# virajmehta/vae-training

Hardware: AMD Instinct MI355X
Metric: ELBO train-step samples/sec (higher is better)
Workload: dtype f32; 1 GPU; M: linear-padding dd3 pad9 (D=12) L=20 linear enc/dec -tdv eps=-1 lr=1e-3 (seed_linpadding_expts.sh:1); batch_per_gpu=65536, global_batch=65536, data_dim=12, latent_dim=20, params=533, parallelism=dp1, grad_exchange=none, launch=direct library call x2395 steps (arguments marshalled once), input_batches=48

## Files before the change

### vae_training_amd/csrc/linear_moments.hip

```cpp
#include <stdlib.h>

#include <type_traits>

#include "comm_dev.h"
#include "rng_dev.h"
#include "vaek_internal.h"

namespace vaek {

using f32x4 = __attribute__((ext_vector_type(4))) float;
using d2 = __attribute__((ext_vector_type(2))) double;
typedef __attribute__((address_space(3))) void lds_void_t;
typedef const __attribute__((address_space(1))) void glb_void_t;

constexpr int LNT = 512, LNW = LNT / 64;
constexpr int kLinMaxPersist = 64;
constexpr int kLinCarry = 2, kLinSlots = kLinMaxPersist + kLinCarry;
struct LinWindow { int first, count; };
struct LinWindows { LinWindow stream, reduce, update; };
constexpr LinWindows lin_windows(int K, int j) {
    const int s0 = kLinMaxPersist * j, s1 = s0 + kLinMaxPersist < K ? s0 + kLinMaxPersist : K;
    const bool last = s1 == K;
    const int r0 = s0 >= 1 ? s0 - 1 : 0, u0 = s0 >= 2 ? s0 - 2 : 0;
    return LinWindows{{s0, s1 - s0}, {r0, (last ? K : s1 - 1) - r0}, {u0, (last ? K : s1 - 2) - u0}};
}
constexpr int lin_launches(int K) { return (K + kLinMaxPersist - 1) / kLinMaxPersist; }
constexpr bool lin_windows_ok(int K) {
    int s = 0, r = 0, u = 0;
    for (int j = 0; j < lin_launches(K); ++j) {
        const LinWindows w = lin_windows(K, j);
        if (w.stream.first != s || w.reduce.first != r || w.update.first != u) return false;
        if (w.stream.count < 1 || w.stream.count > kLinMaxPersist || w.reduce.count < 1 || w.update.count < 1) return false;
        s += w.stream.count; r += w.reduce.count; u += w.update.count;
        if (r > s || u > r || s - w.update.first > kLinSlots) return false;
    }
    return s == K && r == K && u == K;
}
static_assert(lin_windows_ok(1) && lin_windows_ok(2) && lin_windows_ok(64) && lin_windows_ok(65) && lin_windows_ok(66) && lin_windows_ok(128) &&
              lin_windows_ok(129) && lin_windows_ok(130) && lin_windows_ok(960), "launch windows of a vaek_train_steps call");
static_assert(lin_windows(64, 0).update.count == 64 && lin_windows(130, 1).update.first == 62 && lin_windows(130, 1).reduce.first == 63 &&
              lin_windows(130, 2).update.count == 4, "launch windows of a vaek_train_steps call");
constexpr int kLinReduceSets = 1;
constexpr int kLinReduceWgs = 24;

constexpr int kLinCommBanks = 4;
struct LinComm { unsigned long long* peer[kMaxWorld]; int world, rank, ng2; };

constexpr int kLinShards = 8, kLinShardStride = 32;
struct LinPtrs { const float* x[64]; const float* z1[64]; const float* z2[64]; };
struct LinArgs {
    int has_update, n_reduce, n_stream;
    int B, D, L, ntiles, T;
    const float* x; const float* z1; const float* z2; float* partial_out;
    const float* partial_in; double* M_out;
    const double* M_in;
    int persistent, n_steps, sets;
    int n_red, n_str, slot_upd, slot_red, slot_str;
    int d_red, d_str;
    float* partial_base; double* M_base;
    unsigned* cnt_stream; unsigned* cnt_reduce; unsigned* status;
    float* params; float* grads; float* m; float* v; int32_t* step_dev; float lr;
    float inv_bt, eps_cli, rows, rows_over_bt; int off_eps, P;
    float* loss_hist; long long loss_hist_cap;
    int stagger;
    LinComm comm;
};

#ifndef VAEK_LIN_ABL
#define VAEK_LIN_ABL 0
#endif
#ifdef VAEK_LIN_STAMPS
#ifdef VAEK_LIN_FOUR_BLOCK_TU
static __device__ unsigned long long* g_lin_stamp_buf = nullptr;
#else
__device__ unsigned long long* g_lin_stamp_buf = nullptr;
#endif
int lin_stamps_four(unsigned long long* buf);
#define LIN_STAMP(i)                                                                                         \
    do {                                                                                                     \
        if (VAEK_LIN_STAMPS == 2) break;          \
        __builtin_amdgcn_sched_barrier(0);                                                                   \
        unsigned long long _t;                                                                               \
        unsigned long long _r;                                                                               \
        asm volatile("s_waitcnt vmcnt(0) lgkmcnt(0)\n\ts_memtime %0\n\ts_memrealtime %1\n\ts_waitcnt lgkmcnt(0)" : "=s"(_t), "=s"(_r)::"memory"); \
        if (g_lin_stamp_buf && threadIdx.x == 0) { g_lin_stamp_buf[i] = _t; g_lin_stamp_buf[16 + (i)] = _r; } \
        __builtin_amdgcn_sched_barrier(0);                                                                   \
    } while (0)
#define LIN_NOW(v)                                                                                           \
    do {                                                                                                     \
        __builtin_amdgcn_sched_barrier(0);                                                                   \
        if (VAEK_LIN_STAMPS == 2) asm volatile("s_memrealtime %0\n\ts_waitcnt lgkmcnt(0)" : "=s"(v)::"memory");             \
        else asm volatile("s_waitcnt vmcnt(0) lgkmcnt(0)\n\ts_memrealtime %0\n\ts_waitcnt lgkmcnt(0)" : "=s"(v)::"memory"); \
        __builtin_amdgcn_sched_barrier(0);                                                                   \
    } while (0)
#define LIN_NOWQ(v)                                     \
    do {                                                                                                     \
        __builtin_amdgcn_sched_barrier(0);                                                                   \
        asm volatile("s_memrealtime %0\n\ts_waitcnt lgkmcnt(0)" : "=s"(v)::"memory");                        \
        __builtin_amdgcn_sched_barrier(0);                                                                   \
    } while (0)
#define LIN_PUT(i, v) do { if (g_lin_stamp_buf && threadIdx.x == 0) g_lin_stamp_buf[i] = (v); } while (0)
#define LIN_PUTMAX(i, v) do { if (g_lin_stamp_buf && threadIdx.x == 0) atomicMax(&g_lin_stamp_buf[i], (v)); } while (0)
#else
#define LIN_STAMP(i) do {} while (0)
#define LIN_NOW(v) do {} while (0)
#define LIN_NOWQ(v) do {} while (0)
#define LIN_PUT(i, v) do {} while (0)
#define LIN_PUTMAX(i, v) do {} while (0)
#endif

__device__ __forceinline__ void lin_glds16(const void* gsrc, void* lds_wave_base) {
    __builtin_amdgcn_global_load_lds((glb_void_t*)gsrc, (lds_void_t*)lds_wave_base, 16, 0, 0);
}
template <int N> __device__ __forceinline__ void lin_wait_vmcnt() { asm volatile("s_waitcnt vmcnt(%0)" ::"n"(N) : "memory"); }
__device__ __forceinline__ void lin_barrier() { asm volatile("s_waitcnt lgkmcnt(0)\n\ts_barrier" ::: "memory"); }
__device__ __forceinline__ void lin_wait_vmcnt_upto(int n) {
    switch (n) {
        case 1: lin_wait_vmcnt<1>(); break;   case 2: lin_wait_vmcnt<2>(); break;   case 3: lin_wait_vmcnt<3>(); break;
        case 4: lin_wait_vmcnt<4>(); break;   case 5: lin_wait_vmcnt<5>(); break;   case 6: lin_wait_vmcnt<6>(); break;
        case 7: lin_wait_vmcnt<7>(); break;   case 8: lin_wait_vmcnt<8>(); break;   case 9: lin_wait_vmcnt<9>(); break;
        case 10: lin_wait_vmcnt<10>(); break; case 11: lin_wait_vmcnt<11>(); break; case 12: lin_wait_vmcnt<12>(); break;
        case 13: lin_wait_vmcnt<13>(); break; case 14: lin_wait_vmcnt<14>(); break; case 15: lin_wait_vmcnt<15>(); break;
        case 16: lin_wait_vmcnt<16>(); break; case 17: lin_wait_vmcnt<17>(); break; case 18: lin_wait_vmcnt<18>(); break;
        case 19: lin_wait_vmcnt<19>(); break; case 20: lin_wait_vmcnt<20>(); break;
        default: lin_wait_vmcnt<0>(); break;
    }
}

__device__ __host__ constexpr int lin_blk(int NB, int b1, int b2) { return b1 * NB - b1 * (b1 - 1) / 2 + (b2 - b1); }

__device__ __forceinline__ void st_sc1(float* p, float v) { __hip_atomic_store(p, v, __ATOMIC_RELAXED, __HIP_MEMORY_SCOPE_AGENT); }
__device__ __forceinline__ void st_sc1(double* p, double v) { __hip_atomic_store(p, v, __ATOMIC_RELAXED, __HIP_MEMORY_SCOPE_AGENT); }
__device__ __forceinline__ float ld_sc1(const float* p) { return __hip_atomic_load(p, __ATOMIC_RELAXED, __HIP_MEMORY_SCOPE_AGENT); }
__device__ __forceinline__ double ld_sc1(const double* p) { return __hip_atomic_load(p, __ATOMIC_RELAXED, __HIP_MEMORY_SCOPE_AGENT); }

__device__ __forceinline__ void lin_wait_count(const unsigned* cnt, unsigned target, unsigned* status, unsigned tag) {
    if (threadIdx.x == 0) {
        unsigned spins = 0, seen;
        while ((seen = __hip_atomic_load(cnt, __ATOMIC_RELAXED, __HIP_MEMORY_SCOPE_AGENT)) < target) {
            __builtin_amdgcn_s_sleep(16);
            if ((++spins & 1023u) == 0) {
                if (__hip_atomic_load(status, __ATOMIC_RELAXED, __HIP_MEMORY_SCOPE_AGENT)) break;
                if (spins > (1u << 21)) {
                    unsigned expect = 0;
                    __hip_atomic_compare_exchange_strong(status, &expect, 0x80000000u | tag | (seen & 0xffffu), __ATOMIC_RELAXED,
                                                         __ATOMIC_RELAXED, __HIP_MEMORY_SCOPE_AGENT);
                    break;
                }
            }
        }
    }
    __syncthreads();
}

__device__ __forceinline__ void lin_wait_shards(const unsigned* cnt, unsigned target, unsigned* status, unsigned tag) {
    if (threadIdx.x == 0) {
        unsigned spins = 0, seen;
        for (;;) {
            unsigned v[kLinShards];
#pragma unroll
            for (int k = 0; k < kLinShards; ++k) v[k] = __hip_atomic_load(cnt + k * kLinShardStride, __ATOMIC_RELAXED, __HIP_MEMORY_SCOPE_AGENT);
            seen = 0;
#pragma unroll
            for (int k = 0; k < kLinShards; ++k) seen += v[k];
            if (seen >= target) break;
            __builtin_amdgcn_s_sleep(4);
            if ((++spins & 1023u) == 0) {
                if (__hip_atomic_load(status, __ATOMIC_RELAXED, __HIP_MEMORY_SCOPE_AGENT)) break;
                if (spins > (1u << 21)) {
                    unsigned expect = 0;
                    __hip_atomic_compare_exchange_strong(status, &expect, 0x80000000u | tag | (seen & 0xffffu), __ATOMIC_RELAXED,
                                                         __ATOMIC_RELAXED, __HIP_MEMORY_SCOPE_AGENT);
                    break;
                }
            }
        }
    }
    __syncthreads();
}

__device__ __forceinline__ double lin_sum_over_ranks(const LinComm& c, unsigned epoch, int o, double v, unsigned* status) {
    const unsigned long long bits = (unsigned long long)__double_as_longlong(v), tag = (unsigned long long)epoch << 32;
    const long long bank = (long long)(epoch & (kLinCommBanks - 1)) * c.world * c.ng2;
    for (int p = 0; p < c.world; ++p) {
        unsigned long long* q = c.peer[p] + bank + (long long)c.rank * c.ng2 + 2 * o;
        __hip_atomic_store(q, tag | (bits & 0xffffffffull), __ATOMIC_RELAXED, __HIP_MEMORY_SCOPE_SYSTEM);
        __hip_atomic_store(q + 1, tag | (bits >> 32), __ATOMIC_RELAXED, __HIP_MEMORY_SCOPE_SYSTEM);
    }
    const unsigned long long* own = c.peer[c.rank] + bank + 2 * o;
    double sum = 0.0;
    unsigned spins = 0;
    bool dead = false;
    for (int r = 0; r < c.world; ++r) {
        unsigned long long lo = 0, hi = 0;
        for (;;) {
            lo = __hip_atomic_load(own + (long long)r * c.ng2, __ATOMIC_RELAXED, __HIP_MEMORY_SCOPE_SYSTEM);
            hi = __hip_atomic_load(own + (long long)r * c.ng2 + 1, __ATOMIC_RELAXED, __HIP_MEMORY_SCOPE_SYSTEM);
            if (((unsigned)(lo >> 32) == epoch && (unsigned)(hi >> 32) == epoch) || dead) break;
            __builtin_amdgcn_s_sleep(8);
            if ((++spins & 1023u) == 0) {
                if (__hip_atomic_load(status, __ATOMIC_RELAXED, __HIP_MEMORY_SCOPE_AGENT)) dead = true;
                else if (spins > (1u << 21)) {
                    unsigned expect = 0;
                    __hip_atomic_compare_exchange_strong(status, &expect, 0x80000000u | (3u << 28) | ((unsigned)r << 16) | (epoch & 0xffffu),
                                                         __ATOMIC_RELAXED, __ATOMIC_RELAXED, __HIP_MEMORY_SCOPE_AGENT);
                    dead = true;
                }
            }
        }
        sum += __longlong_as_double((long long)((hi << 32) | (lo & 0xffffffffull)));
    }
    return sum;
}

struct LinTile {
    int nz1, nx, np, oX, oZ2, bytes;
    __device__ __host__ LinTile(int D, int L, int T) {
        nz1 = (L * 4 * T + 1023) >> 10; nx = (D * 4 * T + 1023) >> 10; np = nz1 + 2 * nx;
        oX = (nz1 << 10) + 80;
        oZ2 = oX + (nx << 10); bytes = (oZ2 + (nx << 10) + 255) & ~255;
    }
};

__device__ __forceinline__ void lin_issue_piece(const LinArgs& a, const LinTile& tl, const float* x, const float* z1, const float* z2,
                                                int tile, int p, char* slot, int lane) {
    const float* src; int cols, idx, lds_off;
    if (p < tl.nz1) { src = z1; cols = a.L; idx = p; lds_off = 0; }
    else if (p < tl.nz1 + tl.nx) { src = x; cols = a.D; idx = p - tl.nz1; lds_off = tl.oX; }
    else { src = z2; cols = a.D; idx = p - tl.nz1 - tl.nx; lds_off = tl.oZ2; }
    const long long tot = (long long)a.B * cols * 4, base = (long long)tile * a.T * cols * 4;
    const long long last = min(tot & ~15ll, base + (long long)a.T * cols * 4) - 16;
    long long off = base + idx * 1024 + lane * 16;
    off = off <= last ? off : last;
    lin_glds16(reinterpret_cast<const char*>(src) + off, slot + lds_off + idx * 1024);
}

struct LinTileSrc {
    const char *z1, *x, *z2; long long baseL, lastL, baseD, lastD; char* slot; bool on;
    __device__ __forceinline__ void prepare(const LinArgs& a, const float* px, const float* pz1, const float* pz2, int tile, char* slot_) {
        auto uni = [](const float* q) {
            const unsigned long long u = (unsigned long long)q;
            return reinterpret_cast<const char*>((unsigned long long)(unsigned)__builtin_amdgcn_readfirstlane((unsigned)u) |
                                                 ((unsigned long long)(unsigned)__builtin_amdgcn_readfirstlane((unsigned)(u >> 32)) << 32));
        };
        z1 = uni(pz1); x = uni(px); z2 = uni(pz2); slot = slot_; on = true;
        const long long rows = (long long)tile * a.T;
        const long long totL = (long long)a.B * a.L * 4, totD = (long long)a.B * a.D * 4;
        baseL = rows * a.L * 4; baseD = rows * a.D * 4;
        lastL = min(totL & ~15ll, baseL + (long long)a.T * a.L * 4) - 16;
        lastD = min(totD & ~15ll, baseD + (long long)a.T * a.D * 4) - 16;
    }
    __device__ __forceinline__ void issue(const LinTile& tl, int p, int lane) const {
        const char* src; long long base, last; int idx, lds_off;
        if (p < tl.nz1) { src = z1; base = baseL; last = lastL; idx = p; lds_off = 0; }
        else if (p < tl.nz1 + tl.nx) { src = x; base = baseD; last = lastD; idx = p - tl.nz1; lds_off = tl.oX; }
        else { src = z2; base = baseD; last = lastD; idx = p - tl.nz1 - tl.nx; lds_off = tl.oZ2; }
        long long off = base + idx * 1024 + lane * 16;
        off = off <= last ? off : last;
        lin_glds16(src + off, slot + lds_off + idx * 1024);
    }
#pragma clang diagnostic push
#pragma clang diagnostic ignored "-Winline-asm"
    __device__ __forceinline__ void issue_tile(const LinTile& tl, int lw, int NLW, int lane) const {
        auto region = [&](const char* src, long long base, long long last, int n, int lds_off) __attribute__((always_inline)) {
            const long long b2 = base <= last ? base : last;
            const char* sbase = src + b2;
            const unsigned lastrel = (unsigned)(last - b2), degenerate = base <= last ? 0xffffffffu : 0u;
            const unsigned m0_0 = (unsigned)(size_t)(lds_void_t*)(slot + lds_off);
            for (int idx = lw; idx < n; idx += NLW) {
                unsigned off = ((unsigned)idx * 1024u + (unsigned)lane * 16u) & degenerate;
                off = off <= lastrel ? off : lastrel;
                asm volatile("s_mov_b32 m0, %2\n\ts_nop 0\n\tglobal_load_lds_dwordx4 %0, %1" ::"v"(off), "s"(sbase), "s"(m0_0 + (unsigned)idx * 1024u) : "memory", "m0");
            }
        };
        region(z1, baseL, lastL, tl.nz1, 0);
        region(x, baseD, lastD, tl.nx, tl.oX);
        region(z2, baseD, lastD, tl.np - tl.nz1 - tl.nx, tl.oZ2);
    }
#pragma clang diagnostic pop
};

__device__ __forceinline__ void lin_fix_ragged(const LinArgs& a, const LinTile& tl, const float* x, const float* z1, const float* z2,
                                               int tile, char* slot, int t) {
    const int T = a.T;
    const long long row0 = (long long)tile * T;
    const int valid = (int)min((long long)T, (long long)a.B - row0), D = a.D, L = a.L;
    if (valid < T) {
        auto patch_tail = [&](const float* src, int cols, int lds_off) {
            const long long tot = (long long)a.B * cols * 4, full = tot & ~15ll, base = row0 * cols * 4;
            if (t < (int)((tot - full) / 4) && full >= base) reinterpret_cast<float*>(slot + lds_off)[(full - base) / 4 + t] = src[full / 4 + t];
        };
        patch_tail(z1, L, 0); patch_tail(x, D, tl.oX); patch_tail(z2, D, tl.oZ2);
        for (int e = valid * L + t; e < T * L; e += LNT) reinterpret_cast<float*>(slot)[e] = 0.f;
        for (int e = valid * D + t; e < T * D; e += LNT) { reinterpret_cast<float*>(slot + tl.oX)[e] = 0.f; reinterpret_cast<float*>(slot + tl.oZ2)[e] = 0.f; }
    }
    lin_barrier();
}
__device__ __forceinline__ void lin_write_vcol(float* v, int T, int valid, int t) {
    for (int r = t; r < T; r += LNT) v[r] = r < valid ? 1.f : 0.f;
}

__device__ __forceinline__ void st_sc1_x4(float* p, f32x4 v) {
    asm volatile("global_store_dwordx4 %0, %1, off sc1\n\ts_nop 1" ::"v"(p), "v"(v) : "memory");
}

constexpr int lin_scratch_bytes(int NB) { return LNW * (NB * (NB + 1) / 2) * 1024; }
constexpr int lin_ring_scratch_bytes(int NB) { return NB == 3 ? lin_scratch_bytes(NB) : lin_scratch_bytes(NB) / 2; }
constexpr int kLinCW = 4;
template <int NB, int JT, int CW, typename Hook>
__device__ __forceinline__ void lin_tile_products(const LinArgs& a, const LinTile& tl, const char* smem, int slot_off, int v_off, int c_off,
                                                  f32x4 (&acc)[NB * (NB + 1) / 2], int lane, int wave, Hook&& hook) {
    constexpr int NBLK = NB * (NB + 1) / 2;
    const int g = lane >> 4, D = a.D, L = a.L;
    int fb[NB], fs[NB];
#pragma unroll
    for (int u = 0; u < NB; ++u) {
        const int f = 16 * u + (lane & 15);
        if (f < L) { fb[u] = slot_off + f * 4; fs[u] = L * 4; }
        else if (f < L + D) { fb[u] = slot_off + tl.oX + (f - L) * 4; fs[u] = D * 4; }
        else if (f < L + 2 * D) { fb[u] = slot_off + tl.oZ2 + (f - L - D) * 4; fs[u] = D * 4; }
        else if (f == L + 2 * D) { fb[u] = v_off; fs[u] = 4; }
        else { fb[u] = c_off; fs[u] = 0; }
    }
#pragma unroll
    for (int k = 0; k < NBLK; ++k) acc[k] = f32x4{0.f, 0.f, 0.f, 0.f};
    const int J = JT ? JT : a.T / (4 * CW), wbase = (a.T / CW) * wave, jfull = J & ~3;
    auto products = [&](const float (&op)[NB]) __attribute__((always_inline)) {
        int k = 0;
#pragma unroll
        for (int b1 = 0; b1 < NB; ++b1)
#pragma unroll
            for (int b2 = b1; b2 < NB; ++b2, ++k) {
                if (VAEK_LIN_ABL & 2) acc[k][0] += op[b1] * op[b2];
                else acc[k] = __builtin_amdgcn_mfma_f32_16x16x4f32(op[b1], op[b2], acc[k], 0, 0, 0);
            }
    };
    if constexpr (JT > 0) {
        constexpr int JF = JT & ~3;
        int cur[NB], fs13[NB], tail[NB];
#pragma unroll
        for (int u = 0; u < NB; ++u) {
            cur[u] = fb[u] + (wbase + 4 * g) * fs[u]; fs13[u] = 13 * fs[u];
            tail[u] = fb[u] + (wbase + 4 * JF + (JT - JF) * g) * fs[u];
        }
        float op[JT][NB];
        auto fetch = [&](int j) __attribute__((always_inline)) {
#pragma unroll
            for (int u = 0; u < NB; ++u) {
                if (j == JF) cur[u] = tail[u];
                op[j][u] = *reinterpret_cast<const float*>(smem + cur[u]);
                cur[u] += (j < JF && (j & 3) == 3) ? fs13[u] : fs[u];
            }
        };
        fetch(0);
        if (JT > 1) fetch(1);
#pragma unroll
        for (int j = 0; j < JT; ++j) {
            if (j + 2 < JT) fetch(j + 2);
            hook(j);
            __builtin_amdgcn_sched_barrier(0);
            products(op[j]);
            __builtin_amdgcn_sched_barrier(0);
        }
    } else {
        float op[2][NB];
        auto fetch = [&](int set, int j) __attribute__((always_inline)) {
            const int sample = wbase + (j < jfull ? 16 * (j >> 2) + (j & 3) + 4 * g : 4 * jfull + (j - jfull) + (J - jfull) * g);
#pragma unroll
            for (int u = 0; u < NB; ++u) op[set][u] = *reinterpret_cast<const float*>(smem + fb[u] + sample * fs[u]);
        };
        fetch(0, 0);
        for (int j = 0; j < J; j += 2) {
            if (j + 1 < J) fetch(1, j + 1);
            hook(j);
            __builtin_amdgcn_sched_barrier(0);
            products(op[0]);
            __builtin_amdgcn_sched_barrier(0);
            if (j + 1 < J) {
                if (j + 2 < J) fetch(0, j + 2);
                hook(j + 1);
                __builtin_amdgcn_sched_barrier(0);
                products(op[1]);
                __builtin_amdgcn_sched_barrier(0);
            }
        }
    }
}

template <int NB, bool SC1, int CW>
__device__ __forceinline__ void lin_tile_combine(const f32x4 (&acc)[NB * (NB + 1) / 2], char* scratch, float* out, int t, int wave, int lane) {
    constexpr int NBLK = NB * (NB + 1) / 2;
    f32x4* scr = reinterpret_cast<f32x4*>(scratch);
    if (wave < CW) {
#pragma unroll
        for (int k = 0; k < NBLK; ++k) scr[(wave * NBLK + k) * 64 + lane] = acc[k];
    }
    lin_barrier();
    for (int q = t; q < NBLK * 64; q += LNT) {
        f32x4 sum = scr[q];
#pragma unroll
        for (int w = 1; w < CW; ++w) sum += scr[w * NBLK * 64 + q];
        if ((VAEK_LIN_ABL & 4) && sum[0] != 12345.f) continue;
        if (SC1) st_sc1_x4(out + 4 * q, sum); else *reinterpret_cast<f32x4*>(out + 4 * q) = sum;
    }
}
__device__ __forceinline__ void lin_img_coords(int e, int& blk, int& i, int& j) {
    blk = e >> 8; const int ln = (e >> 2) & 63; i = ((ln >> 4) << 2) + (e & 3); j = ln & 15;
}

template <bool SC1>
__device__ __forceinline__ void lin_reduce(const float* partial_in, double* M_out, int ntiles, char* smem, int rb, int no,
                                           const LinComm* cm = nullptr, unsigned epoch = 0, unsigned* status = nullptr) {
    double* sums = reinterpret_cast<double*>(smem);
    const int t = threadIdx.x, o = rb * 32 + (t & 31), rg = t >> 5;
    const int rpg = (ntiles + 15) / 16, r_lo = rg * rpg, r_hi = min(ntiles, r_lo + rpg);
    double s = 0.0;
    if (o < no)
        for (int r0 = r_lo; r0 < r_hi; r0 += 16) {
            float tv[16];
#pragma unroll
            for (int u = 0; u < 16; ++u) {
                const float* q = partial_in + (long long)min(r0 + u, r_hi - 1) * no + o;
                tv[u] = SC1 ? ld_sc1(q) : *q;
            }
#pragma unroll
            for (int u = 0; u < 16; ++u) s += r0 + u < r_hi ? (double)tv[u] : 0.0;
        }
    sums[rg * 32 + (t & 31)] = s;
    __syncthreads();
    if (t < 32 && o < no) {
        double tot = 0.0;
#pragma unroll
        for (int k = 0; k < 16; ++k) tot += sums[k * 32 + t];
        if (cm && cm->world > 1) tot = lin_sum_over_ranks(*cm, epoch, o, tot, status);
        if (SC1) st_sc1(M_out + o, tot); else M_out[o] = tot;
    }
}

__device__ __forceinline__ void lin_reduce_pair(const float* partial_in, double* M_out, int ntiles, char* smem, int rb0, int rb1, int no,
                                                const LinComm& cm, unsigned epoch, unsigned* status) {
    double* sums = reinterpret_cast<double*>(smem);
    const int t = threadIdx.x, q = t & 31, rg = t >> 5, o0 = rb0 * 32 + q, o1 = rb1 * 32 + q;
    const int rpg = (ntiles + 15) / 16, r_lo = rg * rpg, r_hi = min(ntiles, r_lo + rpg);
    double s0 = 0.0, s1 = 0.0;
    for (int r0 = r_lo; r0 < r_hi; r0 += 16) {
        float ta[16], tb[16];
#pragma unroll
        for (int u = 0; u < 16; ++u) {
            const float* row = partial_in + (long long)min(r0 + u, r_hi - 1) * no;
            ta[u] = ld_sc1(row + o0); tb[u] = ld_sc1(row + o1);
        }
#pragma unroll
        for (int u = 0; u < 16; ++u) { s0 += r0 + u < r_hi ? (double)ta[u] : 0.0; s1 += r0 + u < r_hi ? (double)tb[u] : 0.0; }
    }
    sums[rg * 32 + q] = s0; sums[512 + rg * 32 + q] = s1;
    __syncthreads();
    if (t < 64) {
        const int which = t >> 5;
        double tot = 0.0;
#pragma unroll
        for (int k = 0; k < 16; ++k) tot += sums[which * 512 + k * 32 + q];
        if (cm.world > 1) tot = lin_sum_over_ranks(cm, epoch, which ? o1 : o0, tot, status);
        st_sc1(M_out + (which ? o1 : o0), tot);
    }
}

constexpr int LKOUT = 4;
template <int NB, int DT, int LT>
struct LinUpd {
    static constexpr int NFP = 16 * NB, NBLK = NB * (NB + 1) / 2;
    int D, L, P, fone, off_be, off_wd, off_bd, off_epsp, off_eps;
    double *Mf, *SM, *P1, *G, *Wed, *Wdd, *bed, *bdd, *sd, *elv, *lvd, *dwd, *red, *epsv;
    float p[LKOUT], m[LKOUT], v[LKOUT];

    __device__ __forceinline__ void carve(const LinArgs& a, char* smem) {
        D = DT ? DT : a.D; L = LT ? LT : a.L; P = a.P; fone = L + 2 * D; off_eps = a.off_eps;
        off_be = D * L; off_wd = off_be + L; off_bd = off_wd + L * D; off_epsp = off_bd + D;
        Mf = reinterpret_cast<double*>(smem);
        SM = Mf + NFP * NFP; P1 = SM + L * NFP; G = P1 + D * NFP;
        Wed = G + L * NFP; Wdd = Wed + D * L; bed = Wdd + L * D; bdd = bed + L; sd = bdd + D; elv = sd + L; lvd = elv + L;
        dwd = lvd + L; red = dwd + L * D; epsv = red + 4 * LNW;
    }
    static __host__ size_t lds_bytes(int D, int L) {
        return sizeof(double) * ((size_t)NFP * NFP + (size_t)(D + 2 * L) * NFP + 3 * (size_t)D * L + 5 * L + D + 4 * LNW + 2);
    }
    __device__ __forceinline__ void load_state(const LinArgs& a) {
        const int t = threadIdx.x;
#pragma unroll
        for (int k = 0; k < LKOUT; ++k) {
            const int idx = min(t + LNT * k, P - 1);
            p[k] = a.params[idx]; m[k] = a.m[idx]; v[k] = a.v[idx];
        }
    }
    __device__ __forceinline__ void publish_params() {
        const int t = threadIdx.x;
#pragma unroll
        for (int k = 0; k < LKOUT; ++k) {
            const int i = t + LNT * k;
            const double pv = (double)p[k];
            if (i < off_be) Wed[i] = pv;
            else if (i < off_wd) bed[i - off_be] = pv;
            else if (i < off_bd) Wdd[i - off_wd] = pv;
            else if (i < off_epsp) bdd[i - off_bd] = pv;
            else if (i < off_epsp + L) { const double sl = exp(0.5 * pv); sd[i - off_epsp] = sl; elv[i - off_epsp] = sl * sl; lvd[i - off_epsp] = pv; }
            else if (i == off_eps) epsv[0] = pv;
        }
    }
    template <bool SC1>
    __device__ __forceinline__ void expand_M(const double* M_in) {
        for (int e = threadIdx.x; e < NBLK * 256; e += LNT) {
            int k, i, j;
            lin_img_coords(e, k, i, j);
            int b1 = 0, rem = k;
            while (rem >= NB - b1) { rem -= NB - b1; ++b1; }
            const int b2 = b1 + rem;
            const double val = SC1 ? ld_sc1(M_in + e) : M_in[e];
            Mf[(16 * b1 + i) * NFP + 16 * b2 + j] = val;
            Mf[(16 * b2 + j) * NFP + 16 * b1 + i] = val;
        }
    }
    static constexpr int MPT = (NBLK * 256 + LNT - 1) / LNT;
    __device__ __forceinline__ void fetch_M(const double* M_in, double (&r)[MPT]) {
#pragma unroll
        for (int k = 0; k < MPT; ++k) r[k] = ld_sc1(M_in + min((int)threadIdx.x + LNT * k, NBLK * 256 - 1));
    }
    __device__ __forceinline__ void scatter_M(const double (&r)[MPT]) {
#pragma unroll
        for (int k = 0; k < MPT; ++k) {
            const int e = threadIdx.x + LNT * k;
            if (e < NBLK * 256) {
                int blk, i, j;
                lin_img_coords(e, blk, i, j);
                int b1 = 0, rem = blk;
                while (rem >= NB - b1) { rem -= NB - b1; ++b1; }
                const int b2 = b1 + rem;
                Mf[(16 * b1 + i) * NFP + 16 * b2 + j] = r[k];
                Mf[(16 * b2 + j) * NFP + 16 * b1 + i] = r[k];
            }
        }
    }
    __device__ __forceinline__ void step(const LinArgs& a, int tstep, float (&gout)[LKOUT]) {
        const int t = threadIdx.x;
        const double eps = off_eps >= 0 ? epsv[0] * (double)a.eps_cli : (double)a.eps_cli;
        const double sigma = exp(0.5 * eps), inv_var = 1.0 / (sigma * sigma);
        LIN_STAMP(1);
        if constexpr (DT > 0 && LT > 0 && (DT % 2 == 0) && (LT % 2 == 0) && LT * (NFP / 2) <= LNT && LT * DT <= LNT / 2) {
            constexpr int HP = NFP / 2;
            {
                const int l = min(t / HP, LT - 1), f = (t % HP) * 2;
                double w[DT + 2]; d2 mv[DT + 2];
                w[0] = sd[l]; mv[0] = *reinterpret_cast<const d2*>(Mf + l * NFP + f);
                w[1] = bed[l]; mv[1] = *reinterpret_cast<const d2*>(Mf + fone * NFP + f);
#pragma unroll
                for (int dd = 0; dd < DT; ++dd) { w[2 + dd] = Wed[dd * LT + l]; mv[2 + dd] = *reinterpret_cast<const d2*>(Mf + (LT + dd) * NFP + f); }
                __builtin_amdgcn_sched_barrier(0);
                d2 s2 = w[0] * mv[0];
#pragma unroll
                for (int k = 1; k < DT + 2; ++k) s2 += w[k] * mv[k];
// ... 1004 lines not shown
        }
        const int valid_last = a.B - (a.ntiles - 1) * a.T;
        lin_write_vcol(reinterpret_cast<float*>(lin_smem + v_off), a.T, a.T, t);
        lin_write_vcol(reinterpret_cast<float*>(lin_smem + vr_off), a.T, valid_last, t);
        if (t == 0) { *reinterpret_cast<float*>(lin_smem + c_off) = 0.f; *reinterpret_cast<unsigned*>(lin_smem + c_off + 8) = 0u; }
        __syncthreads();
        const int per_batch = sid < a.ntiles ? (a.ntiles - sid + S - 1) / S : 0, items = a.n_str * per_batch;
        const bool loader = wave >= kLinCW;
        const int lw = wave - kLinCW;
        constexpr int NLW = LNW - kLinCW;
        auto share = [&](int n) { return lw < n ? (n - lw + NLW - 1) / NLW : 0; };
        const int npw = (GEN || !loader) ? 0 : share(tl.nz1) + share(tl.nx) + share(tl.np - tl.nz1 - tl.nx);
        const int sw = wave < (NO / 4 + 63) / 64 ? 1 : 0;
        struct Pos {
            int idx, n, r, slot, bs;
            __device__ __forceinline__ void advance(int per_batch) {
                ++idx; slot = slot == 2 ? 0 : slot + 1;
                if (++r == per_batch) { r = 0; ++n; bs = bs == kLinSlots - 1 ? 0 : bs + 1; }
            }
        };
        auto pos_tile = [&](const Pos& q) { return sid + q.r * S; };
        Pos p_cur{0, 0, 0, 0, a.slot_str}, p_load{0, 0, 0, 0, a.slot_str}, p_sig{0, 0, 0, 0, a.slot_str};
        LinTileSrc nxt;
        nxt.on = false;
        auto prepare = [&]() __attribute__((always_inline)) {
            if constexpr (!GEN) {
                nxt.on = false;
                if (p_load.idx < items) {
                    const int n = p_load.n;
                    nxt.prepare(a, tab[n], tab[kLinMaxPersist + n], tab[2 * kLinMaxPersist + n], pos_tile(p_load), lin_smem + p_load.slot * stride);
                }
                p_load.advance(per_batch);
            }
        };
        auto issue_pieces = [&]() __attribute__((always_inline)) {
            if constexpr (!GEN) { if (!(VAEK_LIN_ABL & 8) && nxt.on) nxt.issue_tile(tl, lw, NLW, lane); }
        };
        constexpr int GT = NLW * 64;
        [[maybe_unused]] const int gD = DT ? DT : a.D, gL = LT ? LT : a.L, nzb = (gL + gD + 3) / 4;
        [[maybe_unused]] const int nlat = a.T * nzb, xr = (a.T + GT - 1) / GT, npair = nlat / (2 * GT), rem = nlat - 2 * GT * npair;
        [[maybe_unused]] const int gen_rounds = xr + npair + (rem + GT - 1) / GT;
        [[maybe_unused]] const unsigned step0 = (unsigned)(a.step_dev[0] + a.d_str);
        [[maybe_unused]] int g_kind = 0, g_dd = 0, g_did = 0; [[maybe_unused]] float g_noise = 0.f; [[maybe_unused]] unsigned g_tag = 0;
        if constexpr (GEN) { g_kind = src.kind; g_dd = src.dd; g_did = src.did; g_noise = src.noise_std; g_tag = src.tag; }
        auto gen_round = [&](const Pos& q, int k, int gt) __attribute__((always_inline)) {
            if constexpr (GEN) {
                if (q.idx < items && k < gen_rounds) {
                    const uint2 key = make_uint2((unsigned)src.seed, (unsigned)(src.seed >> 32));
                    const long long row_lo = (long long)pos_tile(q) * a.T;
                    const unsigned step = step0 + (unsigned)q.n;
                    char* slot = lin_smem + q.slot * stride;
                    auto put = [&](int z, const float (&n4)[4]) __attribute__((always_inline)) {
                        const int r = z / nzb, q = z - r * nzb, c0 = 4 * q;
                        const bool live = row_lo + r < a.B;
                        const f32x4 v4 = live ? f32x4{n4[0], n4[1], n4[2], n4[3]} : f32x4{0.f, 0.f, 0.f, 0.f};
                        float* z1r = reinterpret_cast<float*>(slot) + r * gL;
                        float* z2r = reinterpret_cast<float*>(slot + tl.oZ2) + r * gD;
                        if (c0 + 3 < gL && gL % 4 == 0) *reinterpret_cast<f32x4*>(z1r + c0) = v4;
                        else if (c0 >= gL && (c0 - gL) + 3 < gD && gD % 4 == 0 && gL % 4 == 0) *reinterpret_cast<f32x4*>(z2r + (c0 - gL)) = v4;
                        else {
#pragma unroll
                            for (int c = 0; c < 4; ++c) {
                                if (c0 + c < gL) z1r[c0 + c] = v4[c];
                                else if (c0 + c < gL + gD) z2r[c0 + c - gL] = v4[c];
                            }
                        }
                    };
                    auto draw = [&](int z, float (&n4)[4]) __attribute__((always_inline)) {
                        const int r = z / nzb;
                        latent_block(src, step, src.row0 + row_lo + r, key, z - r * nzb, n4);
                    };
                    if (k >= xr && k < xr + npair) {
                        const int za = 2 * GT * (k - xr) + gt;
                        float na[4], nb[4];
                        draw(za, na); draw(za + GT, nb);
                        put(za, na); put(za + GT, nb);
                    } else if (k >= xr + npair) {
                        const int z = 2 * GT * npair + GT * (k - xr - npair) + gt;
                        if (z < nlat) {
                            float n4[4];
                            draw(z, n4);
                            put(z, n4);
                        }
                    } else {
                        const int row = gt + GT * k;
                        if (row < a.T) {
                            const long long lrow = row_lo + row, grow = src.row0 + lrow;
                            const bool live = lrow < a.B;
                            float nrm[16];
                            dataset_normals(src, step, grow, key, nrm);
                            float* xr_ = reinterpret_cast<float*>(slot + tl.oX) + row * gD;
                            float inv = 0.f;
                            if (g_kind == 2) {
                                float nsq = 0.f;
#pragma unroll
                                for (int d = 0; d < 16; ++d) if (d < g_dd) nsq = fmaf(nrm[d], nrm[d], nsq);
                                inv = 1.f / sqrtf(nsq);
                            }
                            for (int c0 = 0; c0 < gD; c0 += 4) {
                                float o[4] = {0.f, 0.f, 0.f, 0.f};
                                if (c0 < g_dd) {
#pragma unroll
                                    for (int c = 0; c < 4; ++c) {
                                        const int d = c0 + c;
                                        float v = 0.f;
                                        if (d < g_dd) {
                                            if (g_kind == 0) {
#pragma unroll
                                                for (int kk = 0; kk < 16; ++kk) if (kk < g_did) v = fmaf(Amat[d * g_did + kk], nrm[kk], v);
                                            } else {
#pragma unroll
                                                for (int kk = 0; kk < 16; ++kk) v = (kk == d) ? nrm[kk] : v;
                                                v *= inv;
                                            }
                                        }
                                        o[c] = v;
                                    }
                                }
                                if (g_kind == 0 && g_noise > 0.f) {
                                    float n4[4];
                                    normals4(philox4x32_10(make_uint4((unsigned)grow, (unsigned)((g_did + 3) / 4 + c0 / 4), step, g_tag), key), n4);
#pragma unroll
                                    for (int c = 0; c < 4; ++c) o[c] = fmaf(g_noise, n4[c], o[c]);
                                }
                                const f32x4 v4 = live ? f32x4{o[0], o[1], o[2], o[3]} : f32x4{0.f, 0.f, 0.f, 0.f};
                                if (gD % 4 == 0) *reinterpret_cast<f32x4*>(xr_ + c0) = v4;
                                else {
#pragma unroll
                                    for (int c = 0; c < 4; ++c) if (c0 + c < gD) xr_[c0 + c] = v4[c];
                                }
                            }
                        }
                    }
                }
            }
        };
        [[maybe_unused]] unsigned* const ticket = reinterpret_cast<unsigned*>(lin_smem + c_off + 8);
        auto gen_share = [&](const Pos& q0, const Pos& q1, int nitems) __attribute__((always_inline)) {
            if constexpr (GEN) {
                const unsigned units = (unsigned)gen_rounds * NLW, total = units * (unsigned)nitems;
#pragma unroll 1
                for (;;) {
                    unsigned u = 0;
                    if (lane == 0) u = __hip_atomic_fetch_add(ticket, 1u, __ATOMIC_RELAXED, __HIP_MEMORY_SCOPE_WORKGROUP);
                    u = (unsigned)__builtin_amdgcn_readfirstlane((int)u);
                    if (u >= total) break;
                    const bool second = u >= units;
                    const unsigned v = second ? u - units : u;
                    gen_round(second ? q1 : q0, (int)(v / NLW), (int)(v % NLW) * 64 + lane);
                }
            }
        };
        unsigned* const my_shard = a.cnt_stream + (b & (kLinShards - 1)) * kLinShardStride;
        auto signal = [&]() {
            if (t == 0) __hip_atomic_fetch_add(my_shard + p_sig.bs * kLinShards * kLinShardStride, 1u, __ATOMIC_RELAXED, __HIP_MEMORY_SCOPE_AGENT);
            p_sig.advance(per_batch);
        };
        if constexpr (GEN) {
            Pos q1 = p_load;
            q1.advance(per_batch);
            gen_share(p_load, q1, 2);
            p_load.advance(per_batch); p_load.advance(per_batch);
            lin_barrier();
            if (t == 0) *ticket = 0u;
        } else if (loader) {
            prepare();
            issue_pieces();
            prepare();
            issue_pieces();
        }
        [[maybe_unused]] unsigned long long s0 = 0, s1 = 0, s2 = 0, s3 = 0, s4 = 0, s5 = 0, s6 = 0, sacc_i = 0, sacc_l = 0, sacc_f = 0, sacc_m = 0, sacc_p = 0, sacc_b = 0;
        for (int i = 0; i < items; ++i) {
            LIN_NOWQ(s0);
            lin_wait_vmcnt_upto((i + 1 < items ? npw : 0) + (i >= 1 ? sw : 0));
            LIN_NOWQ(s1);
            lin_barrier();
            LIN_NOWQ(s2);
            if (i >= 3) signal();
            const int n = p_cur.n, tile = pos_tile(p_cur), slot_off = p_cur.slot * stride;
            char* slot = lin_smem + slot_off;
            const bool ragged = tile == a.ntiles - 1 && valid_last < a.T;
            if constexpr (!GEN) {
                if (ragged) lin_fix_ragged(a, tl, tab[n], tab[kLinMaxPersist + n], tab[2 * kLinMaxPersist + n], tile, slot, t);
            }
            LIN_NOWQ(s3);
            f32x4 acc[NB * (NB + 1) / 2];
            if (!loader) lin_tile_products<NB, JT, kLinCW>(a, tl, lin_smem, slot_off, ragged ? vr_off : v_off, c_off, acc, lane, wave, [](int) {});
            if constexpr (GEN) {
                gen_share(p_load, p_load, 1);
                p_load.advance(per_batch);
            } else if (loader && i > 0) {
                prepare();
                issue_pieces();
            }
            LIN_NOWQ(s5);
            lin_barrier();
            if constexpr (GEN) { if (t == 0) *ticket = 0u; }
            LIN_NOWQ(s6);
            lin_tile_combine<NB, true, kLinCW>(acc, slot, a.partial_base + ((long long)p_cur.bs * a.ntiles + tile) * NO, t, wave, lane);
            if (i == 0) {
                lin_wait_vmcnt<0>();
                lin_barrier();
                signal();
                if (sid == 0) { [[maybe_unused]] unsigned long long te = 0; LIN_NOWQ(te); LIN_PUT(53, te); }
                if constexpr (!GEN) {
                    if (loader) {
                        prepare();
                        issue_pieces();
                    }
                }
            }
            LIN_NOWQ(s4);
            if (i + 1 < items) { sacc_i += s1 - s0; sacc_l += s2 - s1; sacc_f += s3 - s2; sacc_m += s4 - s3; sacc_p += s5 - s3; sacc_b += s6 - s5; }
            if (sid == 7) { LIN_PUT(42, sacc_i); LIN_PUT(43, sacc_l); LIN_PUT(44, sacc_f); LIN_PUT(45, sacc_m); LIN_PUT(46, (unsigned long long)items); LIN_PUT(47, sacc_p); LIN_PUT(48, sacc_b); }
            p_cur.advance(per_batch);
        }
        lin_wait_vmcnt<0>();
        lin_barrier();
        if (items - 2 >= 1) signal();
        if (items - 1 >= 1) signal();
        { [[maybe_unused]] unsigned long long te = 0; LIN_NOWQ(te); LIN_PUTMAX(49, te); }
    }
}

constexpr unsigned kLinMagic = 0x4c494e33u;
#ifndef VAEK_LIN_FOUR_BLOCK_TU
__global__ void lin_init_kernel(unsigned* cnt, int n_words, unsigned* status) {
    for (int k = threadIdx.x; k < n_words; k += blockDim.x) cnt[k] = 0u;
    if (threadIdx.x == 0 && status[1] != kLinMagic) { status[0] = 0u; status[1] = kLinMagic; }
}
#endif

typedef void (*LinPersistKernel)(const LinArgs, const LinPtrs);
typedef void (*LinPersistGenKernel)(const LinArgs, const BatchArgs);
LinPersistKernel lin_persist_four(int which);
LinPersistGenKernel lin_persist_four_gen(int which);

#ifndef VAEK_LIN_FOUR_BLOCK_TU
constexpr size_t kLinMaxLds = 160 * 1024;
constexpr size_t kLinCntStreamBytes = (size_t)kLinSlots * kLinShards * kLinShardStride * 4, kLinCntBytes = kLinCntStreamBytes + 1024, kLinHeadBytes = kLinCntBytes + 256;
static_assert(kLinSlots * sizeof(unsigned) <= 1024, "cnt_reduce");

LinPlan lin_plan(const vaek_ctx* c) {
    LinPlan p{};
    const int D = c->D, L = c->L;
    p.ok = c->cfg.n_enc_hidden == 0 && c->cfg.n_dec_hidden == 0 && !c->cfg.sigmoid_decoder && c->cfg.dtype == VAEK_F32 &&
           L + 2 * D + 1 <= 64 && (long long)c->B * std::min(D, L) >= 8;
    if (!p.ok) return p;
    p.NB = (L + 2 * D + 1 + 15) / 16 <= 3 ? 3 : 4;
    p.NO = p.NB * (p.NB + 1) / 2 * 256;
    const auto slot_bytes = [&](int T) { return std::max((size_t)LinTile(D, L, T).bytes, (size_t)lin_scratch_bytes(p.NB)); };
    const auto ring_slot_bytes = [&](int T) { return std::max((size_t)LinTile(D, L, T).bytes, (size_t)lin_ring_scratch_bytes(p.NB)); };
    const auto ring_bytes = [&](int T) { return 3 * ring_slot_bytes(T) + 8 * (size_t)T + 16 + 3 * kLinMaxPersist * sizeof(void*) + 64; };
    const auto ksteps_ok = [&](int T) { return (LinTile(D, L, T).np + LNW - kLinCW - 1) / (LNW - kLinCW) <= 18; };
    const int smax = c->n_cu - 1 - kLinReduceSets * kLinReduceWgs;
    const bool upd_ok = p.NB == 3 ? LinUpdM<3, 0, 0>::shape_ok(D, L) : LinUpdMG<4, 0, 0>::shape_ok(D, L);
    p.T = 256;
    if (p.NB == 3) {
        if (smax >= 16 && c->B > 256 * smax) {
            const int T = 32 * (int)(((long long)c->B + 32ll * smax - 1) / (32ll * smax));
            if (T <= 512 && ksteps_ok(T) && ring_bytes(T) <= kLinMaxLds) p.T = T;
        }
    } else if (upd_ok && smax >= 16) {
        int T = 256;
        while (T > 32 && !(ksteps_ok(T) && ring_bytes(T) <= kLinMaxLds)) T -= 32;
        p.T = T;
    }
    p.ntiles = (c->B + p.T - 1) / p.T;
    const size_t upd = std::max(p.NB == 3 ? LinUpd<3, 0, 0>::lds_bytes(D, L) : LinUpd<4, 0, 0>::lds_bytes(D, L),
                                p.NB == 3 ? LinUpdM<3, 0, 0>::lds_bytes(D, L, (int)c->P) : LinUpdMG<4, 0, 0>::lds_bytes(D, L, (int)c->P));
    p.lds_step = std::max(slot_bytes(p.T) + 4 * (size_t)p.T + 16, std::max(upd, (size_t)2 * 16 * 32 * sizeof(double))) + 64;
    p.lds_persist = std::max(std::max(p.lds_step, ring_bytes(p.T)), (size_t)82 * 1024);
    p.persist = upd_ok && p.lds_persist <= kLinMaxLds && ksteps_ok(p.T) && smax >= 16;
    if (p.persist) {
        const int per = (p.ntiles + smax - 1) / smax;
        p.n_stream = (p.ntiles + per - 1) / per;
        p.n_reduce = kLinReduceSets * std::min(kLinReduceWgs, p.NO / 32);
    }
    p.which_persist = p.NB == 3 ? (D == 12 && L == 20 && p.T == 288 ? 0 : 1) : (D == 20 && L == 20 && p.T == 192 ? 3 : 2);
    p.which_step = D == 12 && L == 20 ? 2 : p.NB - 3;
    const int slots = p.persist ? kLinSlots : 2;
    p.M_off = kLinHeadBytes;
    p.partial_off = p.M_off + (size_t)slots * p.NO * sizeof(double) + 256;
    p.ws_bytes = (p.partial_off + (size_t)slots * p.ntiles * p.NO * sizeof(float) + 256 + 255) / 256 * 256;
    if (c->cfg.world > 1 && p.persist) p.comm_bytes = (size_t)kLinCommBanks * c->cfg.world * 2 * p.NO * sizeof(unsigned long long);
    return p;
}

bool lin_steps_supported(const vaek_ctx* c) {
    return c->lin.ok && (c->cfg.world == 1 || (c->lin.persist && c->comm.ready && c->comm.lin_bytes > 0));
}
bool lin_steps_gen_supported(const vaek_ctx* c, int kind) { return lin_steps_supported(c) && c->lin.persist && (kind == 0 || kind == 2); }

struct LinWs { float* partial; double* M; unsigned* cnt; unsigned* cnt_reduce; unsigned* status; };
static LinWs lin_ws(const vaek_ctx* c, void* ws) {
    char* base = static_cast<char*>(ws) + c->ws_lin;
    LinWs w;
    w.cnt = reinterpret_cast<unsigned*>(base); w.cnt_reduce = reinterpret_cast<unsigned*>(base + kLinCntStreamBytes);
    w.status = reinterpret_cast<unsigned*>(base + kLinCntBytes);
    w.M = reinterpret_cast<double*>(base + c->lin.M_off); w.partial = reinterpret_cast<float*>(base + c->lin.partial_off);
    return w;
}

typedef void (*LinStepKernel)(const LinArgs);
static const LinPersistKernel kLinPersist[] = {lin_persist_kernel<3, 12, 20, 18, false>, lin_persist_kernel<3, 0, 0, 0, false>,
                                                lin_persist_four(0), lin_persist_four(1)};
static const LinPersistGenKernel kLinPersistGen[] = {lin_persist_kernel<3, 12, 20, 18, true>, lin_persist_kernel<3, 0, 0, 0, true>,
                                                     lin_persist_four_gen(0), lin_persist_four_gen(1)};
static const LinStepKernel kLinStep[] = {lin_step_kernel<3, 0, 0>, lin_step_kernel<4, 0, 0>, lin_step_kernel<3, 12, 20>};
template <typename K, size_t N> static int lin_kernel(const K (&table)[N], int which, K* fn) {
    static thread_local PerDeviceOnce attr_set[N];
    if (attr_set[which].need()) {
        VAEK_HIP_CHECK(hipFuncSetAttribute((const void*)table[which], hipFuncAttributeMaxDynamicSharedMemorySize, (int)kLinMaxLds));
        attr_set[which].mark();
    }
    *fn = table[which];
    return VAEK_OK;
}

static void lin_fill_common(const vaek_ctx* c, LinArgs& a, float* params, float* grads, float* m, float* v, int32_t* step_dev, float lr) {
    a.B = c->B; a.D = c->D; a.L = c->L; a.T = c->lin.T; a.ntiles = c->lin.ntiles;
    a.params = params; a.grads = grads; a.m = m; a.v = v; a.step_dev = step_dev; a.lr = lr;
    const double rows = c->cfg.world > 1 ? (double)c->Bt : (double)c->B;
    a.inv_bt = (float)(1.0 / (double)c->Bt); a.eps_cli = c->cfg.eps_cli; a.rows = (float)rows;
    a.rows_over_bt = (float)(rows / (double)c->Bt); a.off_eps = (int)c->off_eps; a.P = (int)c->P;
    a.comm = LinComm{};
    a.comm.world = 1;
    if (c->cfg.world > 1 && c->comm.ready && c->comm.lin_bytes > 0) {
        a.comm.world = c->cfg.world; a.comm.rank = c->cfg.rank; a.comm.ng2 = 2 * c->lin.NO;
        for (int r = 0; r < c->cfg.world; ++r)
            a.comm.peer[r] = reinterpret_cast<unsigned long long*>(static_cast<char*>(c->comm.peers[r]) + c->comm.lin_off);
    }
    a.loss_hist = c->loss_hist; a.loss_hist_cap = c->loss_hist_cap;
    static const int stagger = getenv("VAEK_LIN_STAGGER") ? atoi(getenv("VAEK_LIN_STAGGER")) : 3;
    a.stagger = stagger;
}

static int lin_ensure_init(vaek_ctx* c, const LinWs& w, void* ws, hipStream_t st) {
    if (c->lin_ws_ready == ws) return VAEK_OK;
    hipStreamCaptureStatus cap = hipStreamCaptureStatusNone;
    VAEK_HIP_CHECK(hipStreamIsCapturing(st, &cap));
    hipLaunchKernelGGL(lin_init_kernel, dim3(1), dim3(1024), 0, st, w.cnt, (int)(kLinCntBytes / 4), w.status);
    VAEK_HIP_CHECK(hipGetLastError());
    c->lin_ws_issued = ws;
    c->lin_ws_ready = cap == hipStreamCaptureStatusNone ? ws : nullptr;
    return VAEK_OK;
}

static int lin_train_steps_impl(vaek_ctx* c, float* params, float* grads, float* m, float* v, int32_t* step_dev, const float* const* xs,
                                const float* const* z1s, const float* const* z2s, const BatchArgs* gen, int n_steps, float lr, void* ws, hipStream_t st) {
    const LinPlan& p = c->lin;
    const LinWs w = lin_ws(c, ws);
    static const char* env = getenv("VAEK_LIN_PERSIST");
    static const int roles = getenv("VAEK_LIN_ROLES") ? atoi(getenv("VAEK_LIN_ROLES")) : 7;
    const bool persistent = p.persist && (gen || c->cfg.world > 1 || !(env && atoi(env) == 0));
    if (gen && !persistent) { set_error("vaek_train_steps_gen: this context has no persistent form"); return VAEK_ERR_INVALID; }
    if (persistent) {
        LinPersistKernel fn = nullptr;
        LinPersistGenKernel fng = nullptr;
        if (int rc = gen ? lin_kernel(kLinPersistGen, p.which_persist, &fng) : lin_kernel(kLinPersist, p.which_persist, &fn)) return rc;
        if (int rc = lin_ensure_init(c, w, ws, st)) return rc;
        for (int j = 0; j < lin_launches(n_steps); ++j) {
            const LinWindows win = lin_windows(n_steps, j);
            const int s0 = win.stream.first, n = win.stream.count;
            LinArgs a{};
            lin_fill_common(c, a, params, grads, m, v, step_dev, lr);
            a.persistent = 1; a.n_steps = win.update.count; a.n_red = win.reduce.count; a.n_str = n;
            a.slot_upd = win.update.first % kLinSlots; a.slot_red = win.reduce.first % kLinSlots; a.slot_str = s0 % kLinSlots;
            a.d_red = win.reduce.first - win.update.first; a.d_str = s0 - win.update.first;
            a.sets = kLinReduceSets;
            a.has_update = 1; a.n_reduce = p.n_reduce; a.n_stream = p.n_stream;
            if (!(roles & 4)) a.has_update = 0;
            if (!(roles & 2)) { a.has_update = 0; a.n_reduce = 0; }
            if (!(roles & 1)) a.n_stream = 0;
// ... 96 lines not shown
```

Baseline: 18.65 billion samples/s.

## Hand off per-wave moment partials through LDS to loader waves for pipelined combine

Adds a HANDOFF path for the non-generating persistent linear-moments kernel. Compute waves write their accumulator blocks into spare regions of the consumed input slot. The loader waves then sum those partials across waves and store them to global memory one iteration later, overlapping the cross-wave reduction with the next tile's products. A bare barrier placed inside the product loop (at j=VAEK_LIN_K0) acts as the rendezvous, and signalling moves to the loader thread. This is meant to remove the serialized scratch combine and its barrier from the compute waves' critical path. The cost is more complex barrier choreography and reuse of slot memory.

```diff
diff --git a/vae_training_amd/csrc/linear_moments.hip b/vae_training_amd/csrc/linear_moments.hip
--- a/vae_training_amd/csrc/linear_moments.hip
+++ b/vae_training_amd/csrc/linear_moments.hip
@@ -99,12 +99,19 @@
         asm volatile("s_memrealtime %0\n\ts_waitcnt lgkmcnt(0)" : "=s"(v)::"memory");                        \
         __builtin_amdgcn_sched_barrier(0);                                                                   \
     } while (0)
+#define LIN_CLK(t, r)   \
+    do {                                                                                                     \
+        __builtin_amdgcn_sched_barrier(0);                                                                   \
+        asm volatile("s_memtime %0\n\ts_memrealtime %1\n\ts_waitcnt lgkmcnt(0)" : "=s"(t), "=s"(r)::"memory"); \
+        __builtin_amdgcn_sched_barrier(0);                                                                   \
+    } while (0)
 #define LIN_PUT(i, v) do { if (g_lin_stamp_buf && threadIdx.x == 0) g_lin_stamp_buf[i] = (v); } while (0)
 #define LIN_PUTMAX(i, v) do { if (g_lin_stamp_buf && threadIdx.x == 0) atomicMax(&g_lin_stamp_buf[i], (v)); } while (0)
 #else
 #define LIN_STAMP(i) do {} while (0)
 #define LIN_NOW(v) do {} while (0)
 #define LIN_NOWQ(v) do {} while (0)
+#define LIN_CLK(t, r) do {} while (0)
 #define LIN_PUT(i, v) do {} while (0)
 #define LIN_PUTMAX(i, v) do {} while (0)
 #endif
@@ -404,6 +411,20 @@
         if (SC1) st_sc1_x4(out + 4 * q, sum); else *reinterpret_cast<f32x4*>(out + 4 * q) = sum;
     }
 }
+template <int NB, int DT, int LT, int JT>
+struct LinPut {
+    static constexpr int NBLK = NB * (NB + 1) / 2, R = 4 * JT, zb = R * LT * 4, xb = R * DT * 4;
+    static constexpr int nA = zb / 1024 < NBLK ? zb / 1024 : NBLK, nB = xb / 1024 < NBLK - nA ? xb / 1024 : NBLK - nA, nC = NBLK - nA - nB;
+    static constexpr bool fits = JT > 0 && DT > 0 && LT > 0 && nC <= xb / 1024;
+    static __device__ __forceinline__ int off(const LinTile& tl, int w, int k) {
+        return k < nA ? w * zb + k * 1024 : k < nA + nB ? tl.oX + w * xb + (k - nA) * 1024 : tl.oZ2 + w * xb + (k - nA - nB) * 1024;
+    }
+};
+#ifndef VAEK_LIN_K0
+#define VAEK_LIN_K0 4
+#endif
+__device__ __forceinline__ void lin_barrier_bare() { asm volatile("s_barrier" ::: "memory"); }
+
 __device__ __forceinline__ void lin_img_coords(int e, int& blk, int& i, int& j) {
     blk = e >> 8; const int ln = (e >> 2) & 63; i = ((ln >> 4) << 2) + (e & 3); j = ln & 15;
 }
@@ -1714,8 +1735,10 @@
             }
         };
         unsigned* const my_shard = a.cnt_stream + (b & (kLinShards - 1)) * kLinShardStride;
+        constexpr bool HANDOFF = !GEN && LinPut<NB, DT, LT, JT>::fits;
+        constexpr int sig_t = HANDOFF ? kLinCW * 64 : 0;
         auto signal = [&]() {
-            if (t == 0) __hip_atomic_fetch_add(my_shard + p_sig.bs * kLinShards * kLinShardStride, 1u, __ATOMIC_RELAXED, __HIP_MEMORY_SCOPE_AGENT);
+            if (t == sig_t) __hip_atomic_fetch_add(my_shard + p_sig.bs * kLinShards * kLinShardStride, 1u, __ATOMIC_RELAXED, __HIP_MEMORY_SCOPE_AGENT);
             p_sig.advance(per_batch);
         };
         if constexpr (GEN) {
@@ -1731,6 +1754,87 @@
             prepare();
             issue_pieces();
         }
+        if constexpr (HANDOFF) {
+            using Put = LinPut<NB, DT, LT, JT>;
+            constexpr int NBLK = NB * (NB + 1) / 2, NQ = (NBLK + NLW - 1) / NLW;
+            static_assert(VAEK_LIN_K0 >= 0 && VAEK_LIN_K0 < JT, "the rendezvous sits inside the product loop");
+            const int sq = loader ? share(NBLK) : 0;
+            [[maybe_unused]] unsigned long long s0 = 0, s2 = 0, s3 = 0, s4 = 0, s5 = 0, sacc_l = 0, sacc_f = 0, sacc_m = 0, sacc_p = 0;
+            [[maybe_unused]] unsigned long long c0 = 0, c1 = 0, c2 = 0, c3 = 0, cacc_t = 0, cacc_r = 0;
+            const char* pslot = lin_smem;
+            float* pout = nullptr;
+            if (loader && items > 0) lin_wait_vmcnt_upto(items > 1 ? npw : 0);
+            for (int i = 0; items > 0 && i <= items; ++i) {
+                const bool live = i < items;
+                LIN_NOWQ(s0);
+                lin_barrier();
+                LIN_NOWQ(s2);
+                if (i >= 4) signal();
+                const int n = p_cur.n, tile = pos_tile(p_cur), slot_off = p_cur.slot * stride;
+                char* slot = lin_smem + slot_off;
+                const bool ragged = live && tile == a.ntiles - 1 && valid_last < a.T;
+                if (ragged) lin_fix_ragged(a, tl, tab[n], tab[kLinMaxPersist + n], tab[2 * kLinMaxPersist + n], tile, slot, t);
+                LIN_NOWQ(s3);
+                if (!loader) {
+                    if (live) {
+                        f32x4 acc[NBLK];
+                        LIN_CLK(c0, c1);
+                        lin_tile_products<NB, JT, kLinCW>(a, tl, lin_smem, slot_off, ragged ? vr_off : v_off, c_off, acc, lane, wave,
+                                                          [](int j) { if (j == VAEK_LIN_K0) lin_barrier_bare(); });
+                        LIN_CLK(c2, c3);
+                        cacc_t += c2 - c0; cacc_r += c3 - c1;
+                        if (sid == 7) { LIN_PUT(54, cacc_t); LIN_PUT(55, cacc_r); }
+#pragma unroll
+                        for (int k = 0; k < NBLK; ++k) *reinterpret_cast<f32x4*>(slot + Put::off(tl, wave, k) + lane * 16) = acc[k];
+                    } else lin_barrier_bare();
+                } else {
+                    f32x4 sum[NQ];
+                    if (i >= 1) {
+#pragma unroll
+                        for (int r = 0; r < NQ; ++r) {
+                            const int k = lw + NLW * r;
+                            if (k < NBLK) {
+                                f32x4 img[kLinCW];
+#pragma unroll
+                                for (int w = 0; w < kLinCW; ++w) img[w] = *reinterpret_cast<const f32x4*>(pslot + Put::off(tl, w, k) + lane * 16);
+                                sum[r] = img[0];
+#pragma unroll
+                                for (int w = 1; w < kLinCW; ++w) sum[r] += img[w];
+                            }
+                        }
+                    }
+                    lin_barrier();
+                    if (i >= 1) {
+#pragma unroll
+                        for (int r = 0; r < NQ; ++r) {
+                            const int k = lw + NLW * r;
+                            if (k < NBLK && !((VAEK_LIN_ABL & 4) && sum[r][0] != 12345.f)) st_sc1_x4(pout + (k * 64 + lane) * 4, sum[r]);
+                        }
+                    }
+                    if (i == 1 || !live) lin_wait_vmcnt<0>();
+                }
+                LIN_NOWQ(s5);
+                if (i == 1) {
+                    lin_barrier_bare();
+                    signal();
+                    if (sid == 0) { [[maybe_unused]] unsigned long long te = 0; LIN_NOWQ(te); LIN_PUT(53, te); }
+                }
+                if (loader && live) {
+                    prepare();
+                    issue_pieces();
+                    lin_wait_vmcnt_upto((i >= 1 ? sq : 0) + (i + 2 < items ? npw : 0));
+                }
+                LIN_NOWQ(s4);
+                if (i + 1 < items) { sacc_l += s2 - s0; sacc_f += s3 - s2; sacc_m += s4 - s3; sacc_p += s5 - s3; }
+                if (sid == 7) { LIN_PUT(42, 0ull); LIN_PUT(43, sacc_l); LIN_PUT(44, sacc_f); LIN_PUT(45, sacc_m); LIN_PUT(46, (unsigned long long)items); LIN_PUT(47, sacc_p); LIN_PUT(48, 0ull); }
+                pslot = slot;
+                pout = a.partial_base + ((long long)p_cur.bs * a.ntiles + tile) * NO;
+                if (live) p_cur.advance(per_batch);
+            }
+            lin_barrier();
+            while (p_sig.idx < items) signal();
+            { [[maybe_unused]] unsigned long long te = 0; LIN_NOWQ(te); LIN_PUTMAX(49, te); }
+        } else {
         [[maybe_unused]] unsigned long long s0 = 0, s1 = 0, s2 = 0, s3 = 0, s4 = 0, s5 = 0, s6 = 0, sacc_i = 0, sacc_l = 0, sacc_f = 0, sacc_m = 0, sacc_p = 0, sacc_b = 0;
         for (int i = 0; i < items; ++i) {
             LIN_NOWQ(s0);
@@ -1782,6 +1886,7 @@
         if (items - 2 >= 1) signal();
         if (items - 1 >= 1) signal();
         { [[maybe_unused]] unsigned long long te = 0; LIN_NOWQ(te); LIN_PUTMAX(49, te); }
+        }
     }
 }
 
```

Result: slower. 17.87 billion samples/s (-4.2%).
